# lkeegan/blockCG

Hardware: AMD Instinct MI355X
Metric: SBCGrQ lattice-site iterations/sec (iterations/sec x global volume), fp64 (higher is better)
Workload: dtype f64; 1 GPU; SBCGrQ V=64x64x64x64 (64x64x64x64 per GPU), m=16, 4 shifts, mass=0.001, fixed-work (eps=0); m=16, transport=none, half_volume_solves=False, memory_ladder_rung=whole tmp

## Files before the change

blockcg_amd/csrc/kernels_stencil.hip:

```cpp
#include <cassert>

#include "hop_layout.hpp"
#include "hop_plan.hpp"
#include "mfma_common.hpp"

namespace bcg {

namespace {

typedef __attribute__((address_space(3))) char lds_char_t;
__device__ __forceinline__ unsigned lds_addr_of(const void* p) {
  return static_cast<unsigned>(reinterpret_cast<uintptr_t>((lds_char_t*)p));
}
#ifndef BCG_HOP4B_SPREAD
#define BCG_HOP4B_SPREAD 6
#endif
#ifndef BCG_HOP4B_BCAST
#define BCG_HOP4B_BCAST 1
#endif
__device__ __forceinline__ void glds16_link(const void* gsrc, unsigned lds_dst) {
  unsigned keep;
  asm volatile("s_mov_b32 %0, m0\n\ts_mov_b32 m0, %2\n\ts_nop 0\n\tglobal_load_lds_dwordx4 %1, off\n\ts_mov_b32 m0, %0"
               : "=&s"(keep)
               : "v"(gsrc), "s"(lds_dst));
}
__device__ __forceinline__ void glds16(const void* gsrc, unsigned lds_dst) {
  unsigned keep;
  asm volatile("s_mov_b32 %0, m0\n\ts_mov_b32 m0, %2\n\ts_nop 0\n\tglobal_load_lds_dwordx4 %1, off\n\ts_mov_b32 m0, %0"
               : "=&s"(keep)
               : "v"(gsrc), "s"(lds_dst));
}
#ifndef BCG_HOP4B_GLDS_SBASE
#define BCG_HOP4B_GLDS_SBASE 0
#endif
#if BCG_HOP4B_GLDS_SBASE
__device__ __forceinline__ void glds16_s(const char* sbase, unsigned voff, unsigned lds_dst) {
  unsigned keep;
  const unsigned long long a = reinterpret_cast<unsigned long long>(sbase);
  const unsigned lo = __builtin_amdgcn_readfirstlane(static_cast<unsigned>(a));
  const unsigned hi = __builtin_amdgcn_readfirstlane(static_cast<unsigned>(a >> 32));
  const unsigned long long sb = (static_cast<unsigned long long>(hi) << 32) | lo;
  asm volatile("s_nop 4\n\ts_mov_b32 %0, m0\n\ts_mov_b32 m0, %3\n\ts_nop 0\n\tglobal_load_lds_dwordx4 %1, %2\n\ts_mov_b32 m0, %0"
               : "=&s"(keep)
               : "v"(voff), "s"(sb), "s"(lds_dst));
}
#else
__device__ __forceinline__ void glds16_s(const char* sbase, unsigned voff, unsigned lds_dst) { glds16_link(sbase + voff, lds_dst); }
#endif
template <int IMM>
__device__ __forceinline__ dv2 ld_sv_async(const char* sbase, unsigned voff) {
  dv2 r;
  asm volatile("global_load_dwordx4 %0, %1, %2 offset:%3" : "=v"(r) : "v"(voff), "s"(sbase), "n"(IMM));
  return r;
}
template <int LANE, bool NEG>
__device__ __forceinline__ void fmac_bcast(double& acc, double u, double p) {
  if (NEG) asm("v_fmac_f64_dpp %0, -%1, %2 row_newbcast:%3 row_mask:0xf bank_mask:0xf" : "+v"(acc) : "v"(u), "v"(p), "n"(LANE));
  else asm("v_fmac_f64_dpp %0, %1, %2 row_newbcast:%3 row_mask:0xf bank_mask:0xf" : "+v"(acc) : "v"(u), "v"(p), "n"(LANE));
}

__device__ __forceinline__ void wait_vmcnt(int n) {
  switch (n) {
#define BCG_W(k) case k: asm volatile("s_waitcnt vmcnt(" #k ")" ::: "memory"); break;
    BCG_W(1) BCG_W(2) BCG_W(3) BCG_W(4) BCG_W(5) BCG_W(6) BCG_W(7) BCG_W(8) BCG_W(9) BCG_W(10) BCG_W(11) BCG_W(12)
    BCG_W(13) BCG_W(14) BCG_W(15) BCG_W(16) BCG_W(17) BCG_W(18) BCG_W(19) BCG_W(20)
#undef BCG_W
    default: asm volatile("s_waitcnt vmcnt(0)" ::: "memory"); break;
  }
}
__device__ __forceinline__ dv2 ld_link(const dv2* p) { return *p; }
__device__ __forceinline__ void st_nt(double2* p, double2 v) {
  dv2 w;
  w.x = v.x;
  w.y = v.y;
  __builtin_nontemporal_store(w, reinterpret_cast<dv2*>(p));
}

struct TileGeom {
  int x0b, x1, x2, x3;
  int site0;
  int edge;
};

struct HopWalk {
  int p0, p1, p2;
  int xcd_split;
  unsigned* sync;
  int sync_window, sync_stride, sync_limit;
  const int* tile_list;
  int list_n;
  GramFold fold;
  int super;
};

__device__ __forceinline__ unsigned read_counter(unsigned* ctr, unsigned zero) {
  return __hip_atomic_fetch_add(ctr, zero, __ATOMIC_RELAXED, __HIP_MEMORY_SCOPE_AGENT);
}

struct Digits {
  int d0, d1, d2, d3, d4, d5, d6;
};
// ... 607 lines not shown
        double2 t[3] = {make_double2(0, 0), make_double2(0, 0), make_double2(0, 0)};
#pragma unroll
        for (int k = 0; k < 3; ++k) {
#pragma unroll
          for (int r = 0; r < 3; ++r) {
            const double2 u = uf[k * 3 + r];
            t[r].x = fma(u.x, f[mu][k].x, t[r].x); t[r].x = fma(-u.y, f[mu][k].y, t[r].x);
            t[r].y = fma(u.x, f[mu][k].y, t[r].y); t[r].y = fma(u.y, f[mu][k].x, t[r].y);
            const double2 v = ub[r * 3 + k];
            t[r].x = fma(-v.x, bk[mu][k].x, t[r].x); t[r].x = fma(-v.y, bk[mu][k].y, t[r].x);
            t[r].y = fma(-v.x, bk[mu][k].y, t[r].y); t[r].y = fma(v.y, bk[mu][k].x, t[r].y);
          }
        }
#pragma unroll
        for (int r = 0; r < 3; ++r) {
          acc[r].x = fma(eta, t[r].x, acc[r].x);
          acc[r].y = fma(eta, t[r].y, acc[r].y);
        }
        BCG_STAMP(3 + mu)
      }
      double2 tv[3];
#pragma unroll
      for (int r = 0; r < 3; ++r) {
        if (MODE == HOP_PLAIN) tv[r] = make_double2(0.5 * acc[r].x, 0.5 * acc[r].y);
        else tv[r] = make_double2(fma(c0, pv[r].x, -0.5 * acc[r].x), fma(c0, pv[r].y, -0.5 * acc[r].y));
        st_nt(reinterpret_cast<double2*>(orow + voff + r * M * 16), tv[r]);
      }
      if (GRAM) {
#pragma unroll
        for (int r = 0; r < 3; ++r) gram_step<16>(G, &pv[r], &tv[r]);
      }
      if (hw.sync != nullptr && tid == 0 && step_n < hw.sync_stride)
        __hip_atomic_fetch_add(hw.sync + cls * hw.sync_stride + step_n, 1u, __ATOMIC_RELAXED, __HIP_MEMORY_SCOPE_AGENT);
      if (RING) slot = slot + 1 == win.ring ? 0 : slot + 1;
      BCG_STAMP(7)
    }
  }
#undef BCG_FETCH_LINKS
#ifdef BCG_HOP4C_STAMPS
  if (!GRAM && (tid & 63) == 0) {
    double* o = reinterpret_cast<double*>(partials) + (static_cast<int64_t>(blockIdx.x) * 4 + wave) * 8;
    for (int i = 0; i < 8; ++i) o[i] = static_cast<double>(seg[i]);
  }
#endif
#undef BCG_STAMP
  if (GRAM) {
    if (M == 8) gram_block_store_fold8<NW>(G, smem, partials, tid, hw.fold.out != nullptr);
    else gram_block_store<16, NW>(G, smem, partials, tid, hw.fold.out != nullptr);
    gram_fold<M * M>(hw.fold, partials, tid, NW * 64);
  }
}

template <int M, int MODE, bool GRAM, int CLS, bool RING>
__global__ void __launch_bounds__(256) k_hop4c(LatticeDev lat, const double2* __restrict__ U,
                                               const double2* __restrict__ Ughost, const double2* __restrict__ in,
                                               const double2* __restrict__ ghost, double2* __restrict__ out,
                                               const double2* __restrict__ p, double c0,
                                               double2* __restrict__ partials, HopWalk hw, HopWindow win) {
  hop4c_body<M, MODE, GRAM, CLS, RING>(lat, U, Ughost, in, ghost, out, p, c0, partials, hw, win);
}
template <int M, int MODE, bool GRAM>
__global__ void __launch_bounds__(256) __attribute__((amdgpu_waves_per_eu(2, 2)))
k_hop4c_interior(LatticeDev lat, const double2* __restrict__ U, const double2* __restrict__ Ughost,
                 const double2* __restrict__ in, const double2* __restrict__ ghost, double2* __restrict__ out,
                 const double2* __restrict__ p, double c0, double2* __restrict__ partials, HopWalk hw, HopWindow win) {
  hop4c_body<M, MODE, GRAM, 1, false>(lat, U, Ughost, in, ghost, out, p, c0, partials, hw, win);
}



template <int M, int MODE, bool GRAM, bool RING, bool CB = false>
__device__ __forceinline__ void hop4b_body(const LatticeDev& lat, const double2* __restrict__ U,
                                           const double2* __restrict__ Ughost, const double2* __restrict__ in,
                                           const double2* __restrict__ ghost, double2* __restrict__ out,
                                           const double2* __restrict__ p, double c0, double2* __restrict__ partials,
                                           const HopWalk& hw, const HopWindow& win,
                                           const double2* __restrict__ mats = nullptr, int has_rinv = 0) {
  static_assert(!GRAM || M == 16 || M == 8, "fused Gram accumulation: lane&15 = rhs index (m = 16) or (site parity, rhs) (m = 8)");
  constexpr bool RING_OUT = RING && MODE == HOP_PLAIN;
  constexpr bool RING_IN = RING && MODE == HOP_SHIFTED;
  constexpr bool RESID = MODE == HOP_RESID;
  static_assert(!RESID || (GRAM && !RING), "the residual form accumulates a Gram product and is not ring-addressed");
  constexpr bool FUSEB = MODE == HOP_FACT2B;
  constexpr bool FACT = MODE == HOP_FACT1 || MODE == HOP_FACT2 || FUSEB;
  constexpr bool PLUS_D = MODE == HOP_FACT2 || FUSEB;
  constexpr bool HAS_P = MODE == HOP_SHIFTED || MODE == HOP_RESID;
  constexpr bool SHIFT = HAS_P || FACT;
  static_assert(!FACT || (M == 16 && !RING && !CB), "factored pair: whole full-volume fields at m = 16");
  static_assert(!PLUS_D || GRAM, "factored pair: the second factor carries a Gram product");
  constexpr bool SELF_GRAM = FACT && GRAM && kSelfGramProducts != 4;
  static_assert(!CB || (!RING && !RESID), "checkerboard form: whole-field launches only");
  constexpr int SPW = 64 / M;
  constexpr int NW = 4;
  constexpr int CS = hop4b_row_slot(M);
  constexpr int NFW = hop4b_fwd_links(M);
  constexpr int NBW = hop4b_bwd_links(M, CB);
  constexpr int LSTAGE = NFW + NBW;
  constexpr int RFW = (SPW * 36 + 63) / 64;
  constexpr int RBK = (SPW * 9 + 63) / 64;
  constexpr bool SHARE = hop4b_share_images(M);
  constexpr bool PARTNER = SHARE && !CB;
  constexpr bool PIPE = BCG_HOP4B_PIPE != 0 && hop4b_share_images(M) && !RESID;
  constexpr int HB = 3 * M * 16;
  constexpr int NHD = (HB + 1023) / 1024;
  constexpr int RB = 3 * M * 16;
  constexpr int NH = (2 * M + 63) / 64;
  static_assert(NH == 1, "halo sites fit one wave instruction per colour");
  extern __shared__ __attribute__((aligned(16))) double smem[];
  const int tid = threadIdx.x, lane = tid & 63;
  const int wave = __builtin_amdgcn_readfirstlane(tid >> 6);
  const int e1 = wave & 1, e2 = wave >> 1;
  dv2* const Cbase = reinterpret_cast<dv2*>(smem);
  dv2* const Lbase = Cbase + 2 * NW * CS;
  auto image = [&](int x3, int w) __attribute__((always_inline)) { return Lbase + ((SHARE ? (x3 & 1) : 0) * NW + w) * LSTAGE; };
  const int sw = lane / M, j = lane % M;
  const unsigned voff = static_cast<unsigned>((sw * 3 * M + j) * 16);
  const int co = (sw + 1) * 3 * M + j;
  const bool halo_lane = lane < 2 * M;
  const int hs = (lane / M) & 1, hj = lane % M;
  const int ho = (hs ? (SPW + 1) * 3 * M : 0) + hj;
  const int L0 = lat.L[0], L1 = lat.L[1], L2 = lat.L[2], L3 = lat.L[3];
  const int S1 = L0, S2 = L0 * L1, S3 = L0 * L1 * L2;
  const int sp0 = lat.split[0], sp1 = lat.split[1], sp2 = lat.split[2], sp3 = lat.split[3];
  const int gm0 = static_cast<int>(lat.ghost_off[0][0]), gp0 = static_cast<int>(lat.ghost_off[0][1]);
  const int gm1 = static_cast<int>(lat.ghost_off[1][0]), gp1 = static_cast<int>(lat.ghost_off[1][1]);
  const int gm2 = static_cast<int>(lat.ghost_off[2][0]), gp2 = static_cast<int>(lat.ghost_off[2][1]);
  const int gm3 = static_cast<int>(lat.ghost_off[3][0]), gp3 = static_cast<int>(lat.ghost_off[3][1]);
  const int og0 = lat.origin[0], og1 = lat.origin[1], og2 = lat.origin[2];
  const char* const inb = reinterpret_cast<const char*>(in);
  const char* const ghb = reinterpret_cast<const char*>(ghost);
  GramAcc<16> G;
  if (GRAM) gram_zero(G);
  using vd4 = d4;
  dv2* const Ma = reinterpret_cast<dv2*>(smem) + hop4b_lds_bytes(M, CB) / 16;
  dv2* const Mr = Ma + M * M;
  if constexpr (FUSEB) {
    for (int e = tid; e < M * M; e += NW * 64) {
      const int at = (e % M) * M + e / M;
      const double2 a = mats[e];
      Ma[at] = dv2{a.x, a.y};
      if (has_rinv) {
        const double2 b = mats[M * M + e];
        Mr[at] = dv2{b.x, b.y};
      }
    }
  }

  const int r0 = hw.p0 / SPW, r1 = hw.p1 / 2, r4 = L0 / hw.p0, r5 = L1 / hw.p1, r6 = L2 / hw.p2;
  const int cls = blockIdx.x & 7, idx = blockIdx.x >> 3;
  const int d0 = idx % r0, d1 = (idx / r0) % r1, d2 = idx / (r0 * r1);
  const int ppc = (r4 * r5 * r6) >> 3;
  const int x3_end = win.x3_lo + win.x3_n;

  dv2 rf[RFW], rx, rb1[RBK], rb2[RBK], rb3[RBK];
  rx = dv2{0.0, 0.0};
  const unsigned fo = static_cast<unsigned>(lane) * 16;
  static_assert(RBK <= 2, "backward-link elements per lane");
  const unsigned bo_f0 = static_cast<unsigned>((lane / 9) * 36 + lane % 9) * 16;
  const unsigned bo_f1 = static_cast<unsigned>(((lane + 64) / 9) * 36 + (lane + 64) % 9) * 16;
  const unsigned bo_g0 = static_cast<unsigned>(lane) * 16, bo_g1 = static_cast<unsigned>(lane + 64) * 16;
  const unsigned bo_d0 = bo_g0 - bo_f0, bo_d1 = bo_g1 - bo_f1;
#define BO_F(k) ((k) == 0 ? bo_f0 : bo_f1)
#define BO_SEL(G, k) (BO_F(k) + ((G) ? ((k) == 0 ? bo_d0 : bo_d1) : 0u))
#ifdef BCG_HOP4B_STAMPS
  long long seg[16] = {0, 0, 0, 0, 0, 0, 0, 0, 0, 0, 0, 0, 0, 0, 0, 0};
  long long tlast = __builtin_amdgcn_s_memtime();
// ... 299 lines not shown
        fetch_links(lo, true);
        park_links(lo, true);
      }
    }
    auto row_o = [&](bool k_o, int a_o, int s_o, int x3v, int slotv) __attribute__((always_inline)) {
      return k_o ? ghb + (static_cast<int64_t>(a_o) + static_cast<int64_t>(x3v) * s_o) * RB
                 : inb + (static_cast<int64_t>(a_o) + static_cast<int64_t>(RING_IN ? slotv : x3v) * s_o) * RB;
    };
    constexpr bool INCR = SHARE && !CB;
    constexpr bool INCR_IN = INCR && !RING_IN, INCR_OUT = INCR && !RING_OUT;
    const int64_t id_f = static_cast<int64_t>(S3) * (36 * 16), id_row = static_cast<int64_t>(S3) * RB;
    const char* ik_f = nullptr; const char* ik_l = nullptr; const char* ik_1 = nullptr; const char* ik_2 = nullptr;
    const char* ir_own = nullptr; const char* ir_lft = nullptr; const char* ir_rgt = nullptr;
    const char* iw_own = nullptr; const char* iw_lft = nullptr; const char* iw_rgt = nullptr;
    const char* io_1 = nullptr; const char* io_2 = nullptr; const char* ip_p = nullptr; char* ip_o = nullptr;
    int64_t id_l = 0, id_1 = 0, id_2 = 0, id_lft = 0, id_rgt = 0, id_o1 = 0, id_o2 = 0;
    if (INCR) {
      const int lo = win.x3_lo, xn = lo + 1;
      const char* const ub_ = reinterpret_cast<const char*>(U);
      const char* const ug_ = reinterpret_cast<const char*>(Ughost);
      const int64_t sw0 = static_cast<int64_t>(col) + static_cast<int64_t>(xn) * S3;
      const int64_t f0i = x1 + L1 * (x2 + static_cast<int64_t>(L2) * xn);
      const int64_t face = static_cast<int64_t>(L1) * L2;
      ik_f = ub_ + sw0 * (36 * 16);
      if (!row_start) { ik_l = ik_f - 36 * 16; id_l = id_f; }
      else if (!sp0) { ik_l = ik_f + static_cast<int64_t>(L0 - 1) * (36 * 16); id_l = id_f; }
      else { ik_l = ug_ + (static_cast<int64_t>(gm0) + f0i) * (9 * 16); id_l = face * (9 * 16); }
      {
        const int64_t n1 = static_cast<int64_t>(a_b1) + static_cast<int64_t>(xn) * s_b1;
        ik_1 = k_b1 ? ug_ + n1 * (9 * 16) : ub_ + (n1 * 4 + 1) * (9 * 16);
        id_1 = static_cast<int64_t>(s_b1) * (k_b1 ? 9 * 16 : 36 * 16);
        const int64_t n2 = static_cast<int64_t>(a_b2) + static_cast<int64_t>(xn) * s_b2;
        ik_2 = k_b2 ? ug_ + n2 * (9 * 16) : ub_ + (n2 * 4 + 2) * (9 * 16);
        id_2 = static_cast<int64_t>(s_b2) * (k_b2 ? 9 * 16 : 36 * 16);
      }
      if (INCR_IN) ir_own = inb + sw0 * RB;
      if (!INCR_IN) {}
      else if (!row_start) { ir_lft = ir_own - RB; id_lft = id_row; }
      else if (!sp0) { ir_lft = ir_own + static_cast<int64_t>(L0 - 1) * RB; id_lft = id_row; }
      else { ir_lft = ghb + (static_cast<int64_t>(gm0) + f0i) * RB; id_lft = face * RB; }
      if (!INCR_IN) {}
      else if (!row_end) { ir_rgt = ir_own + static_cast<int64_t>(SPW) * RB; id_rgt = id_row; }
      else if (!sp0) { ir_rgt = ir_own - static_cast<int64_t>(L0 - SPW) * RB; id_rgt = id_row; }
      else { ir_rgt = ghb + (static_cast<int64_t>(gp0) + f0i) * RB; id_rgt = face * RB; }
      if (INCR_IN) {
        int kind, xs, gx3;
        slice_of(L3, 0, kind, xs, gx3);
        row_ptrs3(kind, xs, gx3, iw_own, iw_lft, iw_rgt);
      }
      if (INCR_IN) {
        io_1 = row_o(k_o1, a_o1, s_o1, lo, 0);
        io_2 = row_o(k_o2, a_o2, s_o2, lo, 0);
      }
      id_o1 = static_cast<int64_t>(s_o1) * RB;
      id_o2 = static_cast<int64_t>(s_o2) * RB;
      const int64_t c0s = (static_cast<int64_t>(col) + static_cast<int64_t>(lo) * S3) * RB;
      ip_p = reinterpret_cast<const char*>(p) + c0s;
      if (INCR_OUT) ip_o = reinterpret_cast<char*>(out) + c0s;
    }
    double2 o1[3], o2[3];
    if constexpr (PIPE) {
      dv2 q1[3], q2[3];
      {
        const char* const a1 = INCR_IN ? io_1 : row_o(k_o1, a_o1, s_o1, win.x3_lo, slot);
        const char* const a2 = INCR_IN ? io_2 : row_o(k_o2, a_o2, s_o2, win.x3_lo, slot);
        if (INCR_IN) { io_1 += id_o1; io_2 += id_o2; }
#pragma unroll
        for (int c = 0; c < 3; ++c) {
          const double2 v1 = ld_sv(a1, voff, c * M * 16), v2 = ld_sv(a2, voff, c * M * 16);
          q1[c] = dv2{v1.x, v1.y};
          q2[c] = dv2{v2.x, v2.y};
        }
        asm volatile("" : "+v"(q1[0]), "+v"(q1[1]), "+v"(q1[2]), "+v"(q2[0]), "+v"(q2[1]), "+v"(q2[2]));
      }
      constexpr int nB = 3 + 2 * NHD;
      constexpr int nE = HAS_P ? 3 : (FUSEB ? 4 : 0);
      unsigned qo[4] = {0, 0, 0, 0};
      if constexpr (FUSEB) {
        const int i16 = lane & 15, ic = (i16 >> 2) < 3 ? (i16 >> 2) : 2;
        const unsigned qa0 = static_cast<unsigned>((((i16 & 3) * 3 + ic) * M + (lane >> 4)) * 16);
#pragma unroll
        for (int s = 0; s < 4; ++s) qo[s] = has_rinv ? qa0 + s * 64 : voff + (s < 3 ? s : 2) * M * 16;
      }
      const int nC = CB ? RFW + 4 * RBK : RFW + 1 + (e1 ? 0 : RBK) + (e2 ? 0 : RBK);
      constexpr int nD = 6, nS = 3;
      constexpr int SPREAD = HAS_P ? BCG_HOP4B_SPREAD : 0;
      constexpr bool SP_B = (SPREAD & 1) != 0, SP_C = (SPREAD & 2) != 0, SP_D = (SPREAD & 4) != 0;
      (void)nB;
      for (int x3 = win.x3_lo; x3 < x3_end; ++x3) {
        const bool more = x3 + 1 < x3_end;
        const int slot_n = RING ? (slot + 1 == win.ring ? 0 : slot + 1) : 0;
        const int step_n = vs0 + x3;
        if (hw.sync != nullptr && tid == 0 && pace) {
          const int need = step_n - hw.sync_window;
          const unsigned known = seen2_idx == need ? seen2 : (seen1_idx == need ? seen1 : 0u);
          if (need >= 0 && known < per) {
            unsigned* ctr = hw.sync + cls * hw.sync_stride + need;
            const long long t0 = wall_clock64();
            while (read_counter(ctr, zero_rt) < per) {
              if (wall_clock64() - t0 > hw.sync_limit) {
                pace = false;
                break;
              }
              __builtin_amdgcn_s_sleep(2);
            }
          }
        }
        BCG_STAMPB(0)
        __syncthreads();
        BCG_STAMPB(1)
        const dv2* const Lf = image(x3, wave);
        const dv2* const Lb = Lf + NFW;
        const dv2* const ub1 = (PARTNER && e1) ? image(x3, wave ^ 1) + (sw + 1) * 36 + 9 : Lb + sw * 9;
        const dv2* const ub2 = (PARTNER && e2) ? image(x3, wave ^ 2) + (sw + 1) * 36 + 18 : Lb + (SPW + sw) * 9;
        const int rr = CB ? (x1 + x2 + x3 + win.cb_parity) & 1 : 0;
        const dv2* const Cc = Cbase + (x3 & 1) * NW * CS;
        dv2* const Cn = Cbase + (((x3 + 1) & 1) * NW + wave) * CS;
        dv2 f0[3], b0[3], b3[3], f3[3], lp1[3], lp2[3];
#pragma unroll
        for (int c = 0; c < 3; ++c) b3[c] = Cn[co + c * M];
        asm volatile("" : "+v"(b3[0]), "+v"(b3[1]), "+v"(b3[2]));
        const char* b_own;
        const char* b_lft;
        const char* b_rgt;
        {
          const char* own;
          const char* lft;
          const char* rgt;
          if (INCR_IN && x3 + 1 < L3) {
            own = ir_own; lft = ir_lft; rgt = ir_rgt;
            ir_own += id_row; ir_lft += id_lft; ir_rgt += id_rgt;
          } else if (INCR_IN) {
            own = iw_own; lft = iw_lft; rgt = iw_rgt;
          } else {
            int kind, xs, gx3;
            slice_of(x3 + 1, slot_n, kind, xs, gx3);
            row_ptrs3(kind, xs, gx3, own, lft, rgt);
          }
          b_own = own; b_lft = lft; b_rgt = rgt;
        }
        const unsigned cn = __builtin_amdgcn_readfirstlane(lds_addr_of(Cn));
        static_assert(NHD <= 2, "halo site: at most two DMA instructions");
#define BCG_ROW_PIECE(I)                                                                 \
  {                                                                                      \
    if ((I) == 0) glds16_s(b_own, fo, cn + HB);                                          \
    if ((I) == 1) glds16_s(b_own, fo + 1024, cn + HB + 1024);                            \
    if ((I) == 2) glds16_s(b_own, fo + 2048, cn + HB + 2048);                            \
    if ((I) == 3) {                                                                      \
      if (lane * 16 < HB) {                                                              \
        glds16_s(b_lft, fo, cn);                                                         \
        glds16_s(b_rgt, fo, cn + (SPW + 1) * HB);                                        \
      }                                                                                  \
      if (NHD > 1 && lane * 16 + 1024 < HB) {                                            \
        glds16_s(b_lft, fo + 1024, cn + 1024);                                           \
        glds16_s(b_rgt, fo + 1024, cn + (SPW + 1) * HB + 1024);                          \
      }                                                                                  \
    }                                                                                    \
  }
        BCG_ROW_PIECE(0)
        BCG_ROW_PIECE(1)
        if (!SP_B) { BCG_ROW_PIECE(2) BCG_ROW_PIECE(3) }
        BCG_STAMPB(2)
        const dv2* const Cown = Cc + wave * CS;
        const dv2* const Cp1 = Cc + (wave ^ 1) * CS;
        const dv2* const Cp2 = Cc + (wave ^ 2) * CS;
#pragma unroll
        for (int c = 0; c < 3; ++c) {
          f0[c] = Cown[co + (CB ? rr : 1) * 3 * M + c * M];
          b0[c] = Cown[co + (CB ? rr - 1 : -1) * 3 * M + c * M];
        }
        dv2 own[3];
        if (FACT) {
#pragma unroll
          for (int c = 0; c < 3; ++c) own[c] = Cown[co + c * M];
        }
        const int64_t crow_site = static_cast<int64_t>(col) + static_cast<int64_t>(x3) * S3;
        const char* const prow = INCR ? ip_p : reinterpret_cast<const char*>(p) + crow_site * RB;
        char* const orow = INCR_OUT ? ip_o : reinterpret_cast<char*>(out) + (RING_OUT ? static_cast<int64_t>(col) + static_cast<int64_t>(slot) * S3 : crow_site) * RB;
        if (INCR) ip_p += id_row;
        if (INCR_OUT) ip_o += id_row;
        dv2 pv[3], n1[3], n2[3];
        double2 acc[3] = {make_double2(0, 0), make_double2(0, 0), make_double2(0, 0)};
        const int x0 = CB ? 2 * (x0b + sw) + rr : x0b + sw;
        const int par1 = x0 + og0, par2 = par1 + x1 + og1, par3 = par2 + x2 + og2;
#define BCG_LD(K, UF, UB)                                                                                    \
  {                                                                                                          \
    _Pragma("unroll") for (int r = 0; r < 3; ++r) {                                                          \
      LU[r] = (UF)[(K) * 3 + r];                                                                             \
      LU[3 + r] = (UB)[r * 3 + (K)];                                                                         \
    }                                                                                                        \
  }
#define BCG_FM1(MU, K, R, F, B)                                                                              \
  {                                                                                                          \
    constexpr int ef_ = 9 * (MU) + 3 * (K) + (R), eb_ = 9 * (MU) + 3 * (R) + (K);                            \
    fmac_bcast<ef_ % 16, false>(t[R].x, LQ[ef_ / 16].x, F[K].x);                                             \
    fmac_bcast<ef_ % 16, true>(t[R].x, LQ[ef_ / 16].y, F[K].y);                                              \
    fmac_bcast<ef_ % 16, false>(t[R].y, LQ[ef_ / 16].x, F[K].y);                                             \
    fmac_bcast<ef_ % 16, false>(t[R].y, LQ[ef_ / 16].y, F[K].x);                                             \
    fmac_bcast<eb_ % 16, true>(t[R].x, LQ[3 + eb_ / 16].x, B[K].x);                                          \
    fmac_bcast<eb_ % 16, true>(t[R].x, LQ[3 + eb_ / 16].y, B[K].y);                                          \
    fmac_bcast<eb_ % 16, true>(t[R].y, LQ[3 + eb_ / 16].x, B[K].y);                                          \
    fmac_bcast<eb_ % 16, false>(t[R].y, LQ[3 + eb_ / 16].y, B[K].x);                                         \
  }
#define BCG_FMB(MU, K, F, B) { BCG_FM1(MU, K, 0, F, B) BCG_FM1(MU, K, 1, F, B) BCG_FM1(MU, K, 2, F, B) }
#define BCG_FM(K, F, B)                                                                                      \
  {                                                                                                          \
    _Pragma("unroll") for (int r = 0; r < 3; ++r) {                                                          \
      const dv2 u = LU[r];                                                                                   \
      t[r].x = fma(u.x, F[K].x, t[r].x); t[r].x = fma(-u.y, F[K].y, t[r].x);                                 \
      t[r].y = fma(u.x, F[K].y, t[r].y); t[r].y = fma(u.y, F[K].x, t[r].y);                                  \
      const dv2 v = LU[3 + r];                                                                               \
      t[r].x = fma(-v.x, B[K].x, t[r].x); t[r].x = fma(-v.y, B[K].y, t[r].x);                                \
      t[r].y = fma(-v.x, B[K].y, t[r].y); t[r].y = fma(v.y, B[K].x, t[r].y);                                 \
    }                                                                                                        \
  }
#define BCG_PIPE_DIR(MU, F, B, UF, UB, EXTRA, V0, V1)                                                        \
  {                                                                                                          \
    const int par = (MU) == 0 ? 0 : ((MU) == 1 ? par1 : ((MU) == 2 ? par2 : par3));                         \
    const double eta = (par & 1) ? -1.0 : 1.0;                                                               \
    double2 t[3] = {make_double2(0, 0), make_double2(0, 0), make_double2(0, 0)};                             \
    if (BCAST) {                                                                                             \
      BCG_FMB(MU, 0, F, B)                                                                                   \
      BCG_PIPE_SLOT(V0)                                                                                      \
      BCG_FMB(MU, 1, F, B)                                                                                   \
      BCG_PIPE_SLOT(V1)                                                                                      \
      EXTRA                                                                                                  \
      BCG_FMB(MU, 2, F, B)                                                                                   \
    } else {                                                                                                 \
      BCG_LD(0, UF, UB) BCG_FM(0, F, B)                                                                      \
      BCG_PIPE_SLOT(V0)                                                                                      \
      BCG_LD(1, UF, UB) BCG_FM(1, F, B)                                                                      \
      BCG_PIPE_SLOT(V1)                                                                                      \
      EXTRA                                                                                                  \
      BCG_LD(2, UF, UB) BCG_FM(2, F, B)                                                                      \
    }                                                                                                        \
    _Pragma("unroll") for (int r = 0; r < 3; ++r) {                                                          \
      acc[r].x = fma(eta, t[r].x, acc[r].x);                                                                 \
      acc[r].y = fma(eta, t[r].y, acc[r].y);                                                                 \
    }                                                                                                        \
  }
#define BCG_PIPE_SLOT(V)                     \
  if (SPREAD) {                              \
    __builtin_amdgcn_sched_barrier(0);       \
    V                                        \
    __builtin_amdgcn_sched_barrier(0);       \
  }
#define BCG_LD_LP(LP, CP) { _Pragma("unroll") for (int c = 0; c < 3; ++c) LP[c] = (CP)[co + c * M]; }
#define BCG_PIPE_PIN asm volatile("" : "+v"(acc[0].x), "+v"(acc[0].y), "+v"(acc[1].x), "+v"(acc[1].y), "+v"(acc[2].x), "+v"(acc[2].y))
#define BCG_PIPE_APART(text) asm volatile("; " text : "+v"(acc[0].x), "+v"(acc[0].y), "+v"(acc[1].x), "+v"(acc[1].y), "+v"(acc[2].x), "+v"(acc[2].y))
        constexpr bool BCAST = BCG_HOP4B_BCAST != 0;
        dv2 LU[6];
        const dv2* const uf0 = Lf + (sw + 1) * 36;
        const dv2* const ub0 = CB ? Lb + (3 * SPW + sw) * 9 : Lf + sw * 36;
        const dv2* const ub3 = Lb + (2 * SPW + sw) * 9;
        dv2 LQ[6];
        if (BCAST) {
          const int l16 = lane & 15;
#pragma unroll
          for (int q = 0; q < 3; ++q) {
            const int e = l16 + 16 * q < 36 ? l16 + 16 * q : 35;
            LQ[q] = uf0[e];
            const int d = e / 9, i = e - 9 * d;
            const dv2* const ub = d == 0 ? ub0 : (d == 1 ? ub1 : (d == 2 ? ub2 : ub3));
            LQ[3 + q] = ub[i];
          }
        }
        __builtin_amdgcn_sched_barrier(0);
        BCG_PIPE_DIR(0, f0, b0, uf0, ub0, BCG_LD_LP(lp1, Cp1), if (SP_B) BCG_ROW_PIECE(2), if (SP_B) BCG_ROW_PIECE(3))
        BCG_PIPE_PIN;
        __builtin_amdgcn_sched_barrier(0);
#undef BCG_ROW_PIECE
        BCG_STAMPB(3)
        if (HAS_P) {
          asm volatile("; ASYNC_ISSUE p");
          pv[0] = ld_sv_async<0>(prow, voff);
          pv[1] = ld_sv_async<M * 16>(prow, voff);
          pv[2] = ld_sv_async<2 * M * 16>(prow, voff);
          asm volatile("; ASYNC_ISSUED p");
        }
        dv2 qv[4];
        if (FUSEB) {
          asm volatile("; ASYNC_ISSUE q");
          qv[0] = ld_sv_async<0>(prow, qo[0]);
          qv[1] = ld_sv_async<0>(prow, qo[1]);
          qv[2] = ld_sv_async<0>(prow, qo[2]);
          qv[3] = ld_sv_async<0>(prow, qo[3]);
          asm volatile("; ASYNC_ISSUED q");
        }
        constexpr bool C_PIECES = SP_C && INCR && !CB;
        const unsigned imgn = __builtin_amdgcn_readfirstlane(lds_addr_of(image(x3 + 1, wave)));
#define BCG_LINK_PIECE(I)                                                                                    \
  if (more) {                                                                                                \
    if ((I) == 0) {                                                                                          \
      if (lane < SPW * 36) glds16_s(ik_f, fo, imgn + 36 * 16);                                               \
    }                                                                                                        \
    if ((I) == 1) {                                                                                          \
      if (RFW > 1 && lane + 64 < SPW * 36) glds16_s(ik_f, fo + 1024, imgn + (36 + 64) * 16);                 \
    }                                                                                                        \
    if ((I) == 2) {                                                                                          \
      if (RFW > 2 && lane + 128 < SPW * 36) glds16_s(ik_f, fo + 2048, imgn + (36 + 128) * 16);               \
      if (lane < 9) glds16_s(ik_l, fo, imgn);                                                                \
    }                                                                                                        \
    if ((I) == 3) {                                                                                          \
      if (!e1) {                                                                                             \
        if (lane < SPW * 9) glds16_s(ik_1, BO_SEL(k_b1, 0), imgn + NFW * 16);                                \
        if (RBK > 1 && lane + 64 < SPW * 9) glds16_s(ik_1, BO_SEL(k_b1, 1), imgn + (NFW + 64) * 16);         \
      }                                                                                                      \
      if (!e2) {                                                                                             \
        if (lane < SPW * 9) glds16_s(ik_2, BO_SEL(k_b2, 0), imgn + (NFW + SPW * 9) * 16);                    \
        if (RBK > 1 && lane + 64 < SPW * 9) glds16_s(ik_2, BO_SEL(k_b2, 1), imgn + (NFW + SPW * 9 + 64) * 16); \
      }                                                                                                      \
      ik_f += id_f; ik_l += id_l; ik_1 += id_1; ik_2 += id_2;                                                \
    }                                                                                                        \
  }
        if (C_PIECES) {
        } else if (more) {
          if (CB) {
            dma_links_cb(x3 + 1);
          } else if (INCR) {
            dma_links_at_s(x3 + 1, ik_f, ik_l, ik_1, ik_2);
            ik_f += id_f; ik_l += id_l; ik_1 += id_1; ik_2 += id_2;
          } else {
            dma_links(x3 + 1, false);
          }
        }
        __builtin_amdgcn_sched_barrier(0);
        BCG_STAMPB(4)
#define BCG_C1 if (C_PIECES) { BCG_LINK_PIECE(0) }
#define BCG_C2 if (C_PIECES) { BCG_LINK_PIECE(1) }
        if (e1) { BCG_PIPE_DIR(1, q1, lp1, uf0 + 9, ub1, BCG_LD_LP(lp2, Cp2), BCG_C1, BCG_C2) BCG_PIPE_APART("direction 1, forward row outside the bundle"); }
        else { BCG_PIPE_DIR(1, lp1, q1, uf0 + 9, ub1, BCG_LD_LP(lp2, Cp2), BCG_C1, BCG_C2) BCG_PIPE_APART("direction 1, backward row outside the bundle"); }
        BCG_PIPE_PIN;
        __builtin_amdgcn_sched_barrier(0);
#undef BCG_C1
#undef BCG_C2
        BCG_STAMPB(5)
        const char* const a_n1 = INCR_IN ? io_1 : row_o(k_o1, a_o1, s_o1, x3 + 1, slot_n);
        const char* const a_n2 = INCR_IN ? io_2 : row_o(k_o2, a_o2, s_o2, x3 + 1, slot_n);
        if (INCR_IN) { io_1 += id_o1; io_2 += id_o2; }
#define BCG_NEXT_ROW(TAG, N, A)                          \
  if (more) {                                            \
    asm volatile("; ASYNC_ISSUE " TAG);                  \
    N[0] = ld_sv_async<0>(A, voff);                      \
    N[1] = ld_sv_async<M * 16>(A, voff);                 \
    N[2] = ld_sv_async<2 * M * 16>(A, voff);             \
    asm volatile("; ASYNC_ISSUED " TAG);                 \
  }
        BCG_NEXT_ROW("n1", n1, a_n1)
        if (!SP_D) { BCG_NEXT_ROW("n2", n2, a_n2) }
        __builtin_amdgcn_sched_barrier(0);
        BCG_STAMPB(6)
#define BCG_C3 if (C_PIECES) { BCG_LINK_PIECE(2) }
#define BCG_C4 if (C_PIECES) { BCG_LINK_PIECE(3) }
        if (e2) { BCG_PIPE_DIR(2, q2, lp2, uf0 + 18, ub2, , BCG_C3, BCG_C4) BCG_PIPE_APART("direction 2, forward row outside the bundle"); }
        else { BCG_PIPE_DIR(2, lp2, q2, uf0 + 18, ub2, , BCG_C3, BCG_C4) BCG_PIPE_APART("direction 2, backward row outside the bundle"); }
        BCG_PIPE_PIN;
        __builtin_amdgcn_sched_barrier(0);
        if (SP_D) { BCG_NEXT_ROW("n2", n2, a_n2) }
        __builtin_amdgcn_sched_barrier(0);
#undef BCG_C3
#undef BCG_C4
#undef BCG_LINK_PIECE
#undef BCG_NEXT_ROW
        BCG_STAMPB(7)
        wait_vmcnt(nE + (more ? nC + nD : 0));
        BCG_STAMPB(8)
#pragma unroll
        for (int c = 0; c < 3; ++c) f3[c] = Cn[co + c * M];
        BCG_PIPE_DIR(3, f3, b3, uf0 + 27, ub3, , , )
        BCG_PIPE_PIN;
        __builtin_amdgcn_sched_barrier(0);
#undef BCG_LD
#undef BCG_FM
#undef BCG_FM1
#undef BCG_FMB
#undef BCG_PIPE_DIR
#undef BCG_PIPE_SLOT
#undef BCG_LD_LP
#undef BCG_PIPE_PIN
#undef BCG_PIPE_APART
        BCG_STAMPB(9)
        if (more && !CB) park_u3(x3 + 1);
        double2 tv[3], pw[3];
        if (HAS_P) {
          wait_vmcnt(more ? nC + nD : 0);
          dv2 r0, r1, r2;
          asm volatile("; ASYNC_RETIRE p\n\tv_mov_b64 %0, %6\n\tv_mov_b64 %1, %7\n\tv_mov_b64 %2, %8\n\tv_mov_b64 %3, %9\n\tv_mov_b64 %4, %10\n\tv_mov_b64 %5, %11"
                       : "=&v"(r0.x), "=&v"(r0.y), "=&v"(r1.x), "=&v"(r1.y), "=&v"(r2.x), "=&v"(r2.y)
                       : "v"(pv[0].x), "v"(pv[0].y), "v"(pv[1].x), "v"(pv[1].y), "v"(pv[2].x), "v"(pv[2].y));
          pw[0] = make_double2(r0.x, r0.y);
          pw[1] = make_double2(r1.x, r1.y);
          pw[2] = make_double2(r2.x, r2.y);
        }
        if (FACT) {
#pragma unroll
          for (int r = 0; r < 3; ++r) pw[r] = make_double2(own[r].x, own[r].y);
        }
#pragma unroll
        for (int r = 0; r < 3; ++r) {
          if (!SHIFT) tv[r] = make_double2(0.5 * acc[r].x, 0.5 * acc[r].y);
          else if (PLUS_D) tv[r] = make_double2(fma(c0, pw[r].x, 0.5 * acc[r].x), fma(c0, pw[r].y, 0.5 * acc[r].y));
          else tv[r] = make_double2(fma(c0, pw[r].x, -0.5 * acc[r].x), fma(c0, pw[r].y, -0.5 * acc[r].y));
          if (!FUSEB) st_nt(reinterpret_cast<double2*>(orow + voff + r * M * 16), tv[r]);
        }
        double2 qn[3];
        if constexpr (FUSEB) {
          dv2* const slot_h = Cbase + ((x3 & 1) * NW + wave) * CS;
          dv2* const img_b = image(x3, wave) + NFW;
          static_assert(!FUSEB || NBW >= 2 * 3 * M, "two sites of T fit the backward links of an image");
          auto chunk = [&](int site) __attribute__((always_inline)) {
            return (site & 2) ? img_b + (site & 1) * 3 * M : slot_h + (site & 1) * (SPW + 1) * 3 * M;
          };
          dv2* const tw = chunk(sw);
#pragma unroll
          for (int c = 0; c < 3; ++c) tw[c * M + j] = dv2{tv[c].x, tv[c].y};
          wait_vmcnt(more ? nC + nD : 0);
          dv2 qw[4];
          asm volatile("; ASYNC_RETIRE q\n\tv_mov_b64 %0, %8\n\tv_mov_b64 %1, %9\n\tv_mov_b64 %2, %10\n\tv_mov_b64 %3, %11\n\t"
                       "v_mov_b64 %4, %12\n\tv_mov_b64 %5, %13\n\tv_mov_b64 %6, %14\n\tv_mov_b64 %7, %15"
                       : "=&v"(qw[0].x), "=&v"(qw[0].y), "=&v"(qw[1].x), "=&v"(qw[1].y), "=&v"(qw[2].x), "=&v"(qw[2].y),
                         "=&v"(qw[3].x), "=&v"(qw[3].y)
                       : "v"(qv[0].x), "v"(qv[0].y), "v"(qv[1].x), "v"(qv[1].y), "v"(qv[2].x), "v"(qv[2].y), "v"(qv[3].x),
                         "v"(qv[3].y));
          auto rmul_rows = [&](vd4& AR, vd4& AI, const dv2* x, const dv2* Ml) __attribute__((always_inline)) {
            if constexpr (kGauss3M<16>) {
              vd4 K = vd4{0.0, 0.0, 0.0, 0.0};
#pragma unroll
              for (int s = 0; s < 4; ++s) {
                const dv2 cd = Ml[64 * s + lane];
                K = mfma(x[s].x + x[s].y, cd.x, K);
                AR = mfma_nega(x[s].y, cd.x + cd.y, AR);
                AI = mfma(x[s].x, cd.y - cd.x, AI);
              }
              rmul_gauss_fold(AR, AI, K);
            } else {
#pragma unroll
              for (int s = 0; s < 4; ++s) {
                const dv2 cd = Ml[64 * s + lane];
                AR = mfma(x[s].x, cd.x, AR);
                AR = mfma_nega(x[s].y, cd.y, AR);
              }
#pragma unroll
              for (int s = 0; s < 4; ++s) {
                const dv2 cd = Ml[64 * s + lane];
                AI = mfma(x[s].x, cd.y, AI);
                AI = mfma(x[s].y, cd.x, AI);
              }
            }
          };
          vd4 AR = vd4{0.0, 0.0, 0.0, 0.0}, AI = vd4{0.0, 0.0, 0.0, 0.0};
          if (has_rinv) {
            rmul_rows(AR, AI, qw, Mr);
          } else {
            AR = vd4{qw[0].x, qw[1].x, qw[2].x, qw[3].x};
            AI = vd4{qw[0].y, qw[1].y, qw[2].y, qw[3].y};
          }
          const int i16 = lane & 15, ic = (i16 >> 2) < 3 ? (i16 >> 2) : 2;
          const dv2* const tr = chunk(i16 & 3) + ic * M + (lane >> 4);
          dv2 ta[4];
#pragma unroll
          for (int s = 0; s < 4; ++s) ta[s] = tr[4 * s];
          rmul_rows(AR, AI, ta, Ma);
#pragma unroll
          for (int c = 0; c < 3; ++c) {
            qn[c] = make_double2(AR[c], AI[c]);
            st_nt(reinterpret_cast<double2*>(orow + voff + c * M * 16), qn[c]);
          }
        }
        if (GRAM) {
#pragma unroll
          for (int r = 0; r < 3; ++r) {
            const double2* const self = FUSEB ? &qn[r] : (PLUS_D ? &pw[r] : &tv[r]);
            if constexpr (SELF_GRAM) gram_self_step(G, self);
            else if (FACT) gram_step<16>(G, self, self);
            else gram_step<16>(G, &pw[r], &tv[r]);
          }
        }
        BCG_STAMPB(10)
        __builtin_amdgcn_sched_barrier(0);
        if (more) {
          asm volatile("s_waitcnt vmcnt(%24) ; ASYNC_RETIRE n1 ASYNC_RETIRE n2\n\t"
                       "v_mov_b64 %0, %12\n\tv_mov_b64 %1, %13\n\tv_mov_b64 %2, %14\n\tv_mov_b64 %3, %15\n\tv_mov_b64 %4, %16\n\tv_mov_b64 %5, %17\n\t"
                       "v_mov_b64 %6, %18\n\tv_mov_b64 %7, %19\n\tv_mov_b64 %8, %20\n\tv_mov_b64 %9, %21\n\tv_mov_b64 %10, %22\n\tv_mov_b64 %11, %23"
                       : "=&v"(q1[0].x), "=&v"(q1[0].y), "=&v"(q1[1].x), "=&v"(q1[1].y), "=&v"(q1[2].x), "=&v"(q1[2].y),
                         "=&v"(q2[0].x), "=&v"(q2[0].y), "=&v"(q2[1].x), "=&v"(q2[1].y), "=&v"(q2[2].x), "=&v"(q2[2].y)
                       : "v"(n1[0].x), "v"(n1[0].y), "v"(n1[1].x), "v"(n1[1].y), "v"(n1[2].x), "v"(n1[2].y),
                         "v"(n2[0].x), "v"(n2[0].y), "v"(n2[1].x), "v"(n2[1].y), "v"(n2[2].x), "v"(n2[2].y), "n"(nS)
                       : "memory");
        } else {
          asm volatile("s_waitcnt vmcnt(%0)" : : "n"(nS) : "memory");
        }
        if (hw.sync != nullptr && tid == 0 && step_n < hw.sync_stride)
          __hip_atomic_fetch_add(hw.sync + cls * hw.sync_stride + step_n, 1u, __ATOMIC_RELAXED, __HIP_MEMORY_SCOPE_AGENT);
        seen2 = seen1;
        seen2_idx = seen1_idx;
        if (hw.sync != nullptr && tid == 0 && pace && step_n + 2 >= hw.sync_window) {
          seen1_idx = step_n + 2 - hw.sync_window;
          seen1 = read_counter(hw.sync + cls * hw.sync_stride + seen1_idx, zero_rt);
        }
        if (RING) slot = slot_n;
        BCG_STAMPB(11)
      }
    } else
    for (int x3 = win.x3_lo; x3 < x3_end; ++x3) {
      static_assert(!(FUSEB || (MODE == HOP_FACT1 && GRAM)), "the first factor's Gram product and the fused phase B exist in the pipelined step only");
      const int step_n = vs0 + x3;
      if (hw.sync != nullptr && tid == 0 && pace) {
        const int need = step_n - hw.sync_window;
        const unsigned known = seen2_idx == need ? seen2 : (seen1_idx == need ? seen1 : 0u);
        if (need >= 0 && known < per) {
          unsigned* ctr = hw.sync + cls * hw.sync_stride + need;
          const long long t0 = wall_clock64();
          while (read_counter(ctr, zero_rt) < per) {
            if (wall_clock64() - t0 > hw.sync_limit) {
              pace = false;
              break;
            }
            __builtin_amdgcn_s_sleep(2);
          }
        }
      }
      BCG_STAMPB(0)
      __syncthreads();
      BCG_STAMPB(1)
      if (x3 + 1 < x3_end) {
        if (CB) dma_links_cb(x3 + 1);
        else if (SHARE && INCR) {
          dma_links_at(x3 + 1, ik_f, ik_l, ik_1, ik_2);
          ik_f += id_f; ik_l += id_l; ik_1 += id_1; ik_2 += id_2;
        }
        else if (SHARE) dma_links(x3 + 1, false);
        else fetch_links(x3 + 1, false);
      }
      const dv2* const Lf = image(x3, wave);
      const dv2* const Lb = Lf + NFW;
      const dv2* const ub1 = (PARTNER && e1) ? image(x3, wave ^ 1) + (sw + 1) * 36 + 9 : Lb + sw * 9;
      const dv2* const ub2 = (PARTNER && e2) ? image(x3, wave ^ 2) + (sw + 1) * 36 + 18 : Lb + (SPW + sw) * 9;
      const int rr = CB ? (x1 + x2 + x3 + win.cb_parity) & 1 : 0;
      const dv2* const Cc = Cbase + (x3 & 1) * NW * CS;
      dv2* const Cn = Cbase + (((x3 + 1) & 1) * NW + wave) * CS;
      double2 f[4][3], bk[4][3];
#pragma unroll
      for (int c = 0; c < 3; ++c) { const dv2 v = Cn[co + c * M]; bk[3][c] = make_double2(v.x, v.y); }
      {
        const char* const q_o1 = INCR_IN ? io_1 : row_o(k_o1, a_o1, s_o1, x3, slot);
        const char* const q_o2 = INCR_IN ? io_2 : row_o(k_o2, a_o2, s_o2, x3, slot);
        if (INCR_IN) { io_1 += id_o1; io_2 += id_o2; }
#pragma unroll
        for (int c = 0; c < 3; ++c) o1[c] = ld_sv(q_o1, voff, c * M * 16);
#pragma unroll
        for (int c = 0; c < 3; ++c) o2[c] = ld_sv(q_o2, voff, c * M * 16);
      }
      dv2 hv[3];
      {
        int kind, xs, gx3;
        const char* own;
        const char* hal;
        if (INCR_IN && x3 + 1 < L3) {
          own = ir_own;
          hal = (hs ? ir_rgt : ir_lft) + hj * 16;
          ir_own += id_row; ir_lft += id_lft; ir_rgt += id_rgt;
        } else if (INCR_IN && !GRAM) {
          own = iw_own;
          hal = (hs ? iw_rgt : iw_lft) + hj * 16;
        } else {
          slice_of(x3 + 1, RING ? (slot + 1 == win.ring ? 0 : slot + 1) : 0, kind, xs, gx3);
          row_ptrs(kind, xs, gx3, own, hal);
        }
#pragma unroll
        for (int c = 0; c < 3; ++c) f[3][c] = ld_sv(own, voff, c * M * 16);
#pragma unroll
// ... 295 lines not shown
```

Measured before the change: 392.6 million site-iter/s.

## Prefetch fused phase-B q rows one step ahead and overlap Rinv MFMAs

In the fused second-factor hop (HOP_FACT2B), the q rows for the next x3 step are now loaded one iteration early into registers. The Rinv multiply on them is split into per-k MFMA steps interleaved with the next-row neighbour loads, instead of running after a wait on loads issued in the same iteration. The goal is to hide the latency of the q loads and the Rinv product behind stencil memory traffic. The cost is extra live VGPRs (qc, ARq/AIq/Kq) and more intricate vmcnt accounting, which could lower occupancy or introduce ordering hazards.

```diff
diff --git a/blockcg_amd/csrc/kernels_stencil.hip b/blockcg_amd/csrc/kernels_stencil.hip
--- a/blockcg_amd/csrc/kernels_stencil.hip
+++ b/blockcg_amd/csrc/kernels_stencil.hip
@@ -17,6 +17,9 @@
 #endif
 #ifndef BCG_HOP4B_BCAST
 #define BCG_HOP4B_BCAST 1
+#endif
+#ifndef BCG_FUSEB_Q_AHEAD
+#define BCG_FUSEB_Q_AHEAD 1
 #endif
 __device__ __forceinline__ void glds16_link(const void* gsrc, unsigned lds_dst) {
   unsigned keep;
@@ -790,6 +793,7 @@
   constexpr bool RESID = MODE == HOP_RESID;
   static_assert(!RESID || (GRAM && !RING), "the residual form accumulates a Gram product and is not ring-addressed");
   constexpr bool FUSEB = MODE == HOP_FACT2B;
+  constexpr bool Q_AHEAD = FUSEB && BCG_FUSEB_Q_AHEAD != 0;
   constexpr bool FACT = MODE == HOP_FACT1 || MODE == HOP_FACT2 || FUSEB;
   constexpr bool PLUS_D = MODE == HOP_FACT2 || FUSEB;
   constexpr bool HAS_P = MODE == HOP_SHIFTED || MODE == HOP_RESID;
@@ -1255,6 +1259,13 @@
 #pragma unroll
         for (int s = 0; s < 4; ++s) qo[s] = has_rinv ? qa0 + s * 64 : voff + (s < 3 ? s : 2) * M * 16;
       }
+      dv2 qc[4];
+      if constexpr (Q_AHEAD) {
+#pragma unroll
+        for (int s = 0; s < 4; ++s) qc[s] = *reinterpret_cast<const dv2*>(ip_p + qo[s]);
+        asm volatile("" : "+v"(qc[0]), "+v"(qc[1]), "+v"(qc[2]), "+v"(qc[3]));
+        ip_p += id_row;
+      }
       const int nC = CB ? RFW + 4 * RBK : RFW + 1 + (e1 ? 0 : RBK) + (e2 ? 0 : RBK);
       constexpr int nD = 6, nS = 3;
       constexpr int SPREAD = HAS_P ? BCG_HOP4B_SPREAD : 0;
@@ -1343,10 +1354,12 @@
           b0[c] = Cown[co + (CB ? rr - 1 : -1) * 3 * M + c * M];
         }
         dv2 own[3];
-        if (FACT) {
+        if (FACT && !Q_AHEAD) {
 #pragma unroll
           for (int c = 0; c < 3; ++c) own[c] = Cown[co + c * M];
         }
+        dv2 cdq = dv2{0.0, 0.0};
+        if constexpr (Q_AHEAD) cdq = Mr[lane];
         const int64_t crow_site = static_cast<int64_t>(col) + static_cast<int64_t>(x3) * S3;
         const char* const prow = INCR ? ip_p : reinterpret_cast<const char*>(p) + crow_site * RB;
         char* const orow = INCR_OUT ? ip_o : reinterpret_cast<char*>(out) + (RING_OUT ? static_cast<int64_t>(col) + static_cast<int64_t>(slot) * S3 : crow_site) * RB;
@@ -1452,7 +1465,7 @@
           asm volatile("; ASYNC_ISSUED p");
         }
         dv2 qv[4];
-        if (FUSEB) {
+        if (FUSEB && !Q_AHEAD) {
           asm volatile("; ASYNC_ISSUE q");
           qv[0] = ld_sv_async<0>(prow, qo[0]);
           qv[1] = ld_sv_async<0>(prow, qo[1]);
@@ -1519,8 +1532,45 @@
     N[2] = ld_sv_async<2 * M * 16>(A, voff);             \
     asm volatile("; ASYNC_ISSUED " TAG);                 \
   }
+        vd4 ARq = vd4{0.0, 0.0, 0.0, 0.0}, AIq = vd4{0.0, 0.0, 0.0, 0.0}, Kq = vd4{0.0, 0.0, 0.0, 0.0};
+        auto rinv_kstep = [&](int s) __attribute__((always_inline)) {
+          if constexpr (Q_AHEAD) {
+            __builtin_amdgcn_sched_barrier(0);
+            const dv2 cd = cdq;
+            if (s < 3) cdq = Mr[64 * (s + 1) + lane];
+            if (has_rinv) {
+              if constexpr (kGauss3M<16>) {
+                Kq = mfma(qc[s].x + qc[s].y, cd.x, Kq);
+                ARq = mfma_nega(qc[s].y, cd.x + cd.y, ARq);
+                AIq = mfma(qc[s].x, cd.y - cd.x, AIq);
+              } else {
+                ARq = mfma(qc[s].x, cd.x, ARq);
+                ARq = mfma_nega(qc[s].y, cd.y, ARq);
+                AIq = mfma(qc[s].x, cd.y, AIq);
+                AIq = mfma(qc[s].y, cd.x, AIq);
+              }
+            }
+            __builtin_amdgcn_sched_barrier(0);
+          }
+        };
+        if constexpr (Q_AHEAD) {
+          rinv_kstep(0);
+          BCG_NEXT_ROW("n1", n1, a_n1)
+          rinv_kstep(1);
+          BCG_NEXT_ROW("n2", n2, a_n2)
+          rinv_kstep(2);
+          rinv_kstep(3);
+          if (!has_rinv) {
+            ARq = vd4{qc[0].x, qc[1].x, qc[2].x, qc[3].x};
+            AIq = vd4{qc[0].y, qc[1].y, qc[2].y, qc[3].y};
+          }
+          if constexpr (kGauss3M<16>) {
+            if (has_rinv) rmul_gauss_fold(ARq, AIq, Kq);
+          }
+        } else {
         BCG_NEXT_ROW("n1", n1, a_n1)
         if (!SP_D) { BCG_NEXT_ROW("n2", n2, a_n2) }
+        }
         __builtin_amdgcn_sched_barrier(0);
         BCG_STAMPB(6)
 #define BCG_C3 if (C_PIECES) { BCG_LINK_PIECE(2) }
@@ -1536,7 +1586,7 @@
 #undef BCG_LINK_PIECE
 #undef BCG_NEXT_ROW
         BCG_STAMPB(7)
-        wait_vmcnt(nE + (more ? nC + nD : 0));
+        wait_vmcnt((Q_AHEAD ? 0 : nE) + (more ? nC + nD : 0));
         BCG_STAMPB(8)
 #pragma unroll
         for (int c = 0; c < 3; ++c) f3[c] = Cn[co + c * M];
@@ -1565,6 +1615,10 @@
           pw[1] = make_double2(r1.x, r1.y);
           pw[2] = make_double2(r2.x, r2.y);
         }
+        if (Q_AHEAD) {
+#pragma unroll
+          for (int c = 0; c < 3; ++c) own[c] = Cown[co + c * M];
+        }
         if (FACT) {
 #pragma unroll
           for (int r = 0; r < 3; ++r) pw[r] = make_double2(own[r].x, own[r].y);
@@ -1587,8 +1641,20 @@
           dv2* const tw = chunk(sw);
 #pragma unroll
           for (int c = 0; c < 3; ++c) tw[c * M + j] = dv2{tv[c].x, tv[c].y};
-          wait_vmcnt(more ? nC + nD : 0);
+          if constexpr (!Q_AHEAD) wait_vmcnt(more ? nC + nD : 0);
+          if constexpr (Q_AHEAD) {
+            if (more) {
+              const int st1 = has_rinv ? 64 : M * 16, st2 = 2 * st1, st3 = has_rinv ? 3 * 64 : 2 * M * 16;
+              asm volatile("; ASYNC_ISSUE q");
+              qc[0] = ld_sv_async<0>(prow, qo[0]);
+              qc[1] = ld_sv_async<0>(prow + st1, qo[0]);
+              qc[2] = ld_sv_async<0>(prow + st2, qo[0]);
+              qc[3] = ld_sv_async<0>(prow + st3, qo[0]);
+              asm volatile("; ASYNC_ISSUED q");
+            }
+          }
           dv2 qw[4];
+          if constexpr (!Q_AHEAD)
           asm volatile("; ASYNC_RETIRE q\n\tv_mov_b64 %0, %8\n\tv_mov_b64 %1, %9\n\tv_mov_b64 %2, %10\n\tv_mov_b64 %3, %11\n\t"
                        "v_mov_b64 %4, %12\n\tv_mov_b64 %5, %13\n\tv_mov_b64 %6, %14\n\tv_mov_b64 %7, %15"
                        : "=&v"(qw[0].x), "=&v"(qw[0].y), "=&v"(qw[1].x), "=&v"(qw[1].y), "=&v"(qw[2].x), "=&v"(qw[2].y),
@@ -1622,7 +1688,10 @@
             }
           };
           vd4 AR = vd4{0.0, 0.0, 0.0, 0.0}, AI = vd4{0.0, 0.0, 0.0, 0.0};
-          if (has_rinv) {
+          if constexpr (Q_AHEAD) {
+            AR = ARq;
+            AI = AIq;
+          } else if (has_rinv) {
             rmul_rows(AR, AI, qw, Mr);
           } else {
             AR = vd4{qw[0].x, qw[1].x, qw[2].x, qw[3].x};
@@ -1651,6 +1720,7 @@
         }
         BCG_STAMPB(10)
         __builtin_amdgcn_sched_barrier(0);
+        if constexpr (Q_AHEAD) asm volatile("s_waitcnt vmcnt(%0)" : : "n"(nS) : "memory");
         if (more) {
           asm volatile("s_waitcnt vmcnt(%24) ; ASYNC_RETIRE n1 ASYNC_RETIRE n2\n\t"
                        "v_mov_b64 %0, %12\n\tv_mov_b64 %1, %13\n\tv_mov_b64 %2, %14\n\tv_mov_b64 %3, %15\n\tv_mov_b64 %4, %16\n\tv_mov_b64 %5, %17\n\t"
@@ -1660,6 +1730,8 @@
                        : "v"(n1[0].x), "v"(n1[0].y), "v"(n1[1].x), "v"(n1[1].y), "v"(n1[2].x), "v"(n1[2].y),
                          "v"(n2[0].x), "v"(n2[0].y), "v"(n2[1].x), "v"(n2[1].y), "v"(n2[2].x), "v"(n2[2].y), "n"(nS)
                        : "memory");
+          if constexpr (Q_AHEAD)
+            asm volatile("; ASYNC_RETIRE q" : "+v"(qc[0]), "+v"(qc[1]), "+v"(qc[2]), "+v"(qc[3]));
         } else {
           asm volatile("s_waitcnt vmcnt(%0)" : : "n"(nS) : "memory");
         }
```

New measurement: 404.5 million site-iter/s (median of 6 runs). +3.0%, better.
